# qradiolink/qradiolink

Hardware: AMD Instinct MI355X
Metric: IQ MSamples/sec through RX demod chain (higher is better)
Workload: dtype f32

## Files before the change

### qradiolink_amd/csrc/engine.cpp

```cpp
#include "host_common.hpp"
#include "firdes.hpp"
#include <algorithm>
#include <cmath>
#include <complex>
#include <cstdio>
#include <cstdlib>
#include <cstring>
#include <memory>
#include <new>
#include <string>
#include <mutex>
#include <set>
#include <vector>

using namespace qrl;

static thread_local std::string g_last_error;
int qrl_set_error(int code, const std::string& msg) { g_last_error = msg; return code; }

namespace qrl {
static thread_local bool t_launch_error = false;
hipError_t dyn_lds_limit(const void* kernel, int bytes)
{
    static std::mutex mu;
// ... 120 lines not shown
std::vector<float2> to_f2(const std::vector<std::complex<float>>& v)
{
    std::vector<float2> r(v.size());
    for (size_t i = 0; i < v.size(); ++i) r[i] = make_float2(v[i].real(), v[i].imag());
    return r;
}

struct DecimStage {
    bool used = false, mfma = false, pl = false, pm = false;
    int D = 1, Jpad = 0, variant = DECIM_R4_J12, nt = 0, S = 0;
    DevBuf<float> taps;
    DevBuf<float2> edge, edge_b; uint32_t edge_len = 0;
    int alloc_edge(int B, bool two = false) {
        if (!pl && !pm) return QRL_OK;
        edge_len = (uint32_t)(pm ? decim_pm_edge_len(nt, D) : decim_pl_edge_len(nt, D));
        if (!edge_len) return QRL_OK;
        if (int r = edge.alloc((size_t)B * edge_len)) return r;
        return two ? edge_b.alloc((size_t)B * edge_len) : QRL_OK;
    }
    int plan(const std::vector<float>& h, int D_) {
        used = true; D = D_; nt = (int)h.size();
        if (decim_uses_pm(nt, D)) {
            pm = true;
            return taps.upload(decim_pm_layout(h, D));
        }
        if (decim_uses_pl(nt, D)) {
            pl = true;
            return taps.upload(decim_pl_layout(h, D));
        }
        if (decim_uses_mfma(nt, D)) {
            mfma = true;
// ... 3 lines not shown
            return taps.upload(g);
        }
        const int J = (nt + D - 1) / D;
        const size_t kLds2 = 80 * 1024;
        auto pad = [&](int v) { const int jc = decim_jc(v); return (J + jc - 1) / jc * jc; };
        variant = -1;
        if (J <= 10 && decim_lds_bytes(D, pad(DECIM_R2_J10), DECIM_R2_J10) <= kLds2) variant = DECIM_R2_J10;
        else if (J > 36 && J <= 44 && decim_lds_bytes(D, 44, DECIM_R4_J44) <= kLds2) variant = DECIM_R4_J44;
        else if (decim_lds_bytes(D, pad(DECIM_R4_J12), DECIM_R4_J12) <= kLds2) variant = DECIM_R4_J12;
        else variant = DECIM_R1_J14;
        Jpad = pad(variant);
        if (decim_lds_bytes(D, Jpad, variant) > 160 * 1024) return QRL_ERR_ARG;
        return taps.upload(decim_layout(h, D, Jpad));
    }
    uint32_t lookback() const { return pm ? decim_pm_lookback(nt, D) : pl ? (uint32_t)(((nt + D - 1) / D + 1) * D) : mfma ? (uint32_t)(nt + D) : (uint32_t)(Jpad * D); }
    int launch(DecimParams& p, int B, hipStream_t s, int parity = 0) const {
        p.nt = nt;
        float2* e = parity && edge_b.p ? edge_b.p : edge.p;
        if (pm) { p.pl_taps = taps.p; p.pl_edge = e; p.pl_edge_stride = edge_len; p.pl_edge_cap = edge_len; return launch_decim_pm(p, B, s); }
        if (pl) { p.pl_taps = taps.p; p.pl_edge = e; p.pl_edge_stride = edge_len; p.pl_edge_cap = edge_len; return launch_decim_pl(p, B, s); }
        if (mfma) { p.gtab = taps.p; p.S = S; return launch_decim_mfma(p, B, s); }
        launch_decim(p, B, variant, s);
        return 0;
    }
};

}

struct qrl_demod {
    qrl_ctx* ctx = nullptr;
    qrl_demod_config cfg{};
    hipStream_t stream = nullptr;
    bool own_stream = false;
    hipStream_t tail = nullptr;
    hipStream_t fecs = nullptr;
    hipEvent_t ev_q[2] = {nullptr, nullptr}, ev_fec[2] = {nullptr, nullptr}; bool q_valid[2] = {false, false};
    bool grouped = false, grouped_capable = false, fec_deferred = false; FecParams fec_pending{}; int fec_pending_slot = 0;
    DevBuf<uint64_t> qp_snap;
    hipEvent_t ev_ff = nullptr, ev_tail = nullptr;
    hipStream_t pre = nullptr; hipEvent_t ev_pre = nullptr, ev_fe[2] = {nullptr, nullptr}; bool fe_valid[2] = {false, false}; bool pre_pending = false;
    bool input_resident = false;
    hipEvent_t ev_user[4] = {nullptr, nullptr, nullptr, nullptr};
    bool tail_pending = false;
    bool qpsk_fll = false, fsk4_disc = false;
    bool m17 = false;
    DevBuf<float2> s2g, disc4_taps; DevBuf<float> sym4_taps; int disc4_nt = 0, sym4_nt = 0;
    bool fll_slim = false;
    bool d2f_capable = false, d2f = false; DevBuf<float> d2f_taps;
    bool overlap = false, overlap_capable = false; hipEvent_t ev_tail2[2] = {nullptr, nullptr}; bool tail2_valid[2] = {false, false}; uint64_t call_no = 0;
    enum Family { F_2FSK, F_GMSK, F_QPSK, F_DMR, F_4FSK, F_BPSK, F_DSSS, F_ANALOG } fam = F_2FSK;
    int branches = 2;

    int fe_decim = 1, interp = 1, decim = 1, target = 0, sps_eff = 0;
    bool fm = false;

    DecimStage fe;
// ... 448 lines not shown
{
    if (n > cfg.max_chunk) return qrl_set_error(QRL_ERR_TOO_BIG, "n exceeds max_chunk");
    if ((reinterpret_cast<uintptr_t>(iq) & 15u) || (stride & 1u)) return qrl_set_error(QRL_ERR_ARG, "iq must be 16-byte aligned, stride even");
    const int B = cfg.batch;
    uint32_t* counts = (out && out->counts) ? out->counts : counts_scratch.p;
    hipStream_t cs = overlap ? tail : stream;
    const int slot = (int)(call_no & 1);
    if (overlap) {
        if (tail2_valid[slot]) HIPCHK(hipStreamWaitEvent(stream, ev_tail2[slot], 0));
    } else {
        HIPCHK(hipMemsetAsync(counts, 0, (size_t)B * 4 * sizeof(uint32_t), stream));
    }
    if (loops_family() && q_valid[slot]) HIPCHK(hipStreamWaitEvent(stream, ev_q[slot], 0));
    if (grouped && q_valid[slot ^ 1]) HIPCHK(hipStreamWaitEvent(stream, ev_q[slot ^ 1], 0));
    if (pre_pending) { HIPCHK(hipStreamWaitEvent(stream, ev_pre, 0)); pre_pending = false; }
    const bool use_pre = pre && input_resident;
    const float2* in = reinterpret_cast<const float2*>(iq);
    const float2* hist_old = hist_flip ? hist_b.p : hist_a.p;
    float2* hist_new = hist_flip ? hist_a.p : hist_b.p;

    const uint64_t n_in0 = n_in, n_in1 = n_in + n;
    uint64_t n1_0 = n1, n1_1 = n1;
    RingC r1{s1.p, s1_mask}, r2{s2.p, s2_mask}, r2l{s2l.p, s2_mask}, r2f{s2f.p, s2_mask};
    RingF r2d{s2d.p, s2_mask}, r3{s3.p, s2_mask};

    hipEvent_t ev0 = nullptr, ev1 = nullptr;
    if (profiling) {
        HIPCHK(hipEventCreate(&ev0)); HIPCHK(hipEventCreate(&ev1));
        HIPCHK(hipEventRecord(ev0, stream));
    }
    if (fe.used) {
        n1_1 = decim_count(n_in1, 1, fe_decim);
        DecimParams p{};
        p.in = in; p.in_stride = stride; p.n0 = n_in0; p.n = (uint32_t)n;
        p.hist = hist_old; p.hist_len = hist_len;
        p.out = r1; p.m0 = n1_0; p.m_count = (uint32_t)(n1_1 - n1_0);
        p.taps = fe.taps.p; p.D = fe.D; p.Jpad = fe.Jpad;
        p.rot_enable = 1; rot.fill(p);
        if (use_pre) { p.pre_stream = pre; p.pre_event = ev_pre; }
        if (fe.launch(p, B, stream, use_pre ? slot : 0)) return qrl_set_error(QRL_ERR_HIP, "front-end launch: hipFuncSetAttribute failed");
    }
    if (profiling && fe.used) { HIPCHK(hipEventRecord(ev1, stream)); prof_events.emplace_back(ev0, ev1); }
    const uint64_t src0 = fe.used ? n1_0 : n_in0, src1 = fe.used ? n1_1 : n_in1;
    const uint64_t n2_0 = n2, n2_1 = decim_count(src1, interp, decim);
    if (interp == 1) {
        DecimParams p{};
        if (fe.used) { p.in = nullptr; p.in_ring = r1; }
        else { p.in = in; p.in_stride = stride; p.hist = hist_old; p.hist_len = hist_len;
               p.rot_enable = 1; rot.fill(p); }
        p.n0 = src0; p.n = (uint32_t)(src1 - src0);
        p.out = r2; p.m0 = n2_0; p.m_count = (uint32_t)(n2_1 - n2_0);
        p.taps = first.taps.p; p.D = first.D; p.Jpad = first.Jpad;
        if (d2f) {
            const bool sd = cfg.enable_side_outputs && out;
            Dec2FirParams f{};
            f.d = p; f.taps = d2f_taps.p; f.out = RingC{s2f.p, s2_mask};
            f.port = sd && out->filtered ? reinterpret_cast<float2*>(out->filtered) : nullptr;
            f.port_cap = sd ? out->filtered_cap : 0;
            f.counts = counts;
            launch_dec2_fir(f, B, stream);
        } else {
            if (use_pre && !fe.used) { p.pre_stream = pre; p.pre_event = ev_pre; }
            if (first.launch(p, B, stream, use_pre && !fe.used ? slot : 0)) return qrl_set_error(QRL_ERR_HIP, "first-stage launch: hipFuncSetAttribute failed");
        }
    } else {
        ResampParams p{};
        if (fe.used) { p.in = nullptr; p.in_ring = r1; }
        else { p.in = in; p.in_stride = stride; p.hist = hist_old; p.hist_len = hist_len;
               p.rot_enable = 1; rot.fill(p); }
        p.n0 = src0; p.n = (uint32_t)(src1 - src0);
        p.out = r2; p.q0 = n2_0; p.q_count = (uint32_t)(n2_1 - n2_0);
        p.taps = rs_taps.p; p.I = interp; p.D = decim; p.Jp = rs_Jp;
        if (fam == F_DMR && !m17) {
            const bool sd = cfg.enable_side_outputs && out;
            p.port = sd && out->filtered ? reinterpret_cast<float2*>(out->filtered) : nullptr;
            p.port_cap = sd ? out->filtered_cap : 0;
            p.port_counts = counts;
// ... 7 lines not shown
        if (fe.used) { p.in = nullptr; p.in_ring = r1; }
        else { p.in = in; p.in_stride = stride; p.hist = hist_old; p.hist_len = hist_len;
               p.rot_enable = 1; rot.fill(p); }
        p.n0 = src0; p.n = (uint32_t)(src1 - src0);
        p.out = RingC{s_scope.p, scope_mask}; p.m0 = n_scope; p.m_count = (uint32_t)(ns_1 - n_scope);
        p.taps = scope.taps.p; p.D = scope.D; p.Jpad = scope.Jpad;
        if (scope.launch(p, B, stream)) return qrl_set_error(QRL_ERR_HIP, "scope launch: hipFuncSetAttribute failed");
        launch_ring_store(RingC{s_scope.p, scope_mask}, n_scope, (uint32_t)(ns_1 - n_scope), scope_out, scope_cap, scope_counts, B, stream);
        n_scope = ns_1;
    }
    {
        HistParams h{};
        h.in = in; h.in_stride = stride; h.n0 = n_in0; h.n = (uint32_t)n;
        h.hist_old = hist_old; h.hist_new = hist_new; h.hist_len = hist_len;
        h.rot_enable = 1; rot.fill(h);
        if (pre) { HIPCHK(hipEventRecord(ev_fe[slot], stream)); fe_valid[slot] = true; }
        if (use_pre) {
            if (fe_valid[slot ^ 1]) HIPCHK(hipStreamWaitEvent(pre, ev_fe[slot ^ 1], 0));
            launch_hist_save(h, B, pre);
            HIPCHK(hipEventRecord(ev_pre, pre));
            pre_pending = true;
        } else launch_hist_save(h, B, stream);
        hist_flip = !hist_flip;
    }
    if (overlap) {
        HIPCHK(hipEventRecord(ev_ff, stream));
        HIPCHK(hipStreamWaitEvent(tail, ev_ff, 0));
        HIPCHK(hipMemsetAsync(counts, 0, (size_t)B * 4 * sizeof(uint32_t), tail));
    }
    const uint32_t c2 = (uint32_t)(n2_1 - n2_0);
    const bool side = cfg.enable_side_outputs && out;
    if (fam == F_DSSS || fam == F_ANALOG) {
        if (int rr = fam == F_DSSS ? dsss_stages(n2_0, n2_1, out, counts, side) : analog_stages(n2_0, n2_1, out, counts, side)) return rr;
        HIPCHK(hipGetLastError());
        if (take_launch_error()) return QRL_ERR_HIP;
        n_in = n_in1; n1 = n1_1; n2 = n2_1; ++call_no;
        return QRL_OK;
// ... 373 lines not shown
            if (std::getenv("QRL_CU_MAIN")) { if ((r0 = create_role_stream(&d->stream, 0, "MAIN"))) return r0; }
            else if (std::getenv("QRL_MAIN_PRIO_LOW")) {
                int plo = 0, phi = 0;
                (void)hipDeviceGetStreamPriorityRange(&plo, &phi);
                HIPCHK(hipStreamCreateWithPriority(&d->stream, hipStreamNonBlocking, plo));
            }
            else HIPCHK(hipStreamCreateWithFlags(&d->stream, hipStreamNonBlocking));
            d->own_stream = true;
        }
        int lo = 0, hi = 0;
        (void)hipDeviceGetStreamPriorityRange(&lo, &hi);
        int r1;
        if ((r1 = create_role_stream(&d->tail, hi, "TAIL")) || (r1 = create_role_stream(&d->fecs, lo, "FEC"))) return r1;
        if (d->own_stream && !std::getenv("QRL_NO_PRE")) { if ((r1 = create_role_stream(&d->pre, 0, "PRE"))) return r1; }
    }
    HIPCHK(hipEventCreateWithFlags(&d->ev_ff, hipEventDisableTiming));
    HIPCHK(hipEventCreateWithFlags(&d->ev_pre, hipEventDisableTiming));
    for (auto& e : d->ev_fe) HIPCHK(hipEventCreateWithFlags(&e, hipEventDisableTiming));
    HIPCHK(hipEventCreateWithFlags(&d->ev_tail, hipEventDisableTiming));
    for (auto& e : d->ev_tail2) HIPCHK(hipEventCreateWithFlags(&e, hipEventDisableTiming));
    for (auto& e : d->ev_q) HIPCHK(hipEventCreateWithFlags(&e, hipEventDisableTiming));
    for (auto& e : d->ev_fec) HIPCHK(hipEventCreateWithFlags(&e, hipEventDisableTiming));
    int r = d->build();
    if (r) return r;
    *outp = d.release();
    return QRL_OK;
}
void qrl_demod_destroy(qrl_demod* d) { if (d) { (void)d->sync_all(); delete d; } }

int qrl_demod_reset(qrl_demod* d)
// ... 58 lines not shown
        d->tail2_valid[0] = d->tail2_valid[1] = false;
        return QRL_OK;
    case QRL_OPT_FLL_SLIM:
        if (int rs = d->sync_all()) return rs;
        d->fll_slim = value != 0;
        return QRL_OK;
    case QRL_OPT_GROUPED:
        if (value != 0 && !d->grouped_capable) return qrl_set_error(QRL_ERR_ARG, "the grouped order exists for the gr_demod_qpsk chain only");
        if (int rs = d->sync_all()) return rs;
        d->grouped = value != 0;
        return QRL_OK;
    case QRL_OPT_INPUT_RESIDENT: {
        if (int rs = d->sync_all()) return rs;
        if (value != 0 && d->pre) {
            DecimStage& st = d->fe.used ? d->fe : d->first;
            if (st.edge_len && !st.edge_b.p) if (int r = st.edge_b.alloc((size_t)d->cfg.batch * st.edge_len)) return qrl_set_error(r, "edge scratch");
        }
        d->input_resident = value != 0;
        return QRL_OK;
    }
    case QRL_OPT_UNFUSED_DEC2:
        if (!d->d2f_capable) return qrl_set_error(QRL_ERR_ARG, "this chain has no fused 1:2 decimator + shaping filter");
        if (d->n_in != 0) return qrl_set_error(QRL_ERR_STATE, "QRL_OPT_UNFUSED_DEC2 can only be set before the first sample (the two forms carry different state)");
        d->d2f = value == 0;
        return QRL_OK;
    default:
        return qrl_set_error(QRL_ERR_ARG, "unknown option");
    }
}
int qrl_demod_out_caps(const qrl_demod* d, size_t n, size_t* fcap, size_t* ccap, size_t* bcap)
{
// ... 118 lines not shown
    return QRL_OK;
}
int qrl_demod_set_agc(qrl_demod* d, float attack, float decay)
{
    if (!d || d->fam != qrl_demod::F_ANALOG || (d->an_kind != 1 && d->an_kind != 3)) return QRL_ERR_ARG;
    d->an_attack = attack; d->an_decay = decay;
    return QRL_OK;
}
int qrl_demod_process(qrl_demod* d, const float* iq, size_t stride, size_t n, const qrl_demod_out* out)
{
    if (!d || (!iq && n)) return QRL_ERR_ARG;
    HIPCHK(hipSetDevice(d->ctx->device));
    (void)take_launch_error();
    return d->process(iq, stride, n, out);
}
int qrl_demod_sync(qrl_demod* d)
{
    if (!d) return QRL_ERR_ARG;
    if (int rs = d->sync_all()) return rs;
    return QRL_OK;
}
void* qrl_demod_stream(qrl_demod* d) { return d ? d->stream : nullptr; }
int qrl_demod_internal_streams(qrl_demod* d, void* out[3])
{
    if (!d || !out) return QRL_ERR_ARG;
    out[0] = d->stream; out[1] = d->tail; out[2] = d->fecs;
    return QRL_OK;
}

int qrl_demod_profile(qrl_demod* d, int enable)
// ... 71 lines not shown
```

### qradiolink_amd/csrc/engine.hpp

```cpp
#pragma once
#include <hip/hip_runtime.h>
#include <stdint.h>
#include <vector>

namespace qrl {

hipError_t dyn_lds_limit(const void* kernel, int bytes);
bool take_launch_error();

int create_role_stream(hipStream_t* s, int priority, const char* role);

struct RingC { float2* p; uint32_t mask; };
struct RingF { float* p; uint32_t mask; };
struct RingB { uint8_t* p; uint32_t mask; };

template <class Pp>
__device__ __forceinline__ void rot_select(Pp& c, const Pp& p, uint32_t b)
{
    c = p; c.rot_acc = p.rot_acc_s[b]; c.rot_inc = p.rot_inc_s[b]; c.rot_lo = p.rot_lo + (size_t)b * 512;
}
#define ROT_VIEW(T, PS, P, SRC, B) T P##_ps_; if constexpr (PS) rot_select(P##_ps_, SRC, (uint32_t)(B)); const T& P = (PS) ? P##_ps_ : SRC
std::vector<float2> rot_fine_table(uint64_t inc);
void launch_rot_ps_advance(uint64_t* acc, const uint64_t* inc, int B, uint64_t delta, hipStream_t s);
void launch_rot_ps_fill(uint64_t* acc, uint64_t* inc, float2* lo, int B, int set_acc, uint64_t acc0, uint64_t inc0, const float2* lo0, hipStream_t s);
// ... 7 lines not shown
    uint64_t m0; uint32_t m_count;
    const float* taps;
    int D, Jpad;
    int rot_enable; uint64_t rot_acc; uint64_t rot_inc; uint64_t rot_nbase; const float2* rot_lo;
    uint32_t tiles;
    const float* gtab; int S; int nt; uint32_t magic_blk, magic_seg;
    uint32_t tpw, nchunks; int nhi; int dbg;
    int nld;
    int hist_raw;
    uint32_t out_row_mul_m1, out_row_add;
    const float* pl_taps; int pl_J; uint32_t pl_S, pl_nseg, pl_batch; uint64_t pl_m_begin, pl_m_end;
    int pl_E, pl_R; const float* pl_hraw;
    float2* pl_edge; uint32_t pl_edge_stride, pl_edge_cap; uint64_t pl_edge_ms, pl_edge_me;
    hipStream_t pre_stream; hipEvent_t pre_event;
    const uint64_t* rot_acc_s; const uint64_t* rot_inc_s;
};
struct HistParams {
    const float2* in; size_t in_stride; uint64_t n0; uint32_t n;
    const float2* hist_old; float2* hist_new; uint32_t hist_len;
    int rot_enable; uint64_t rot_acc; uint64_t rot_inc; uint64_t rot_nbase; const float2* rot_lo;
    const uint64_t* rot_acc_s; const uint64_t* rot_inc_s;
};
void launch_decim(const DecimParams& p, int batch, int variant, hipStream_t s);
struct Dec2FirParams { DecimParams d; const float* taps; RingC out; float2* port; size_t port_cap; uint32_t* counts; };
bool dec2_fir_supported(int nt1, int D, int nt2);
uint32_t dec2_fir_lookback();
std::vector<float> dec2_fir_table(const std::vector<float>& h1, const std::vector<float>& h2);
void launch_dec2_fir(const Dec2FirParams& p, int batch, hipStream_t s);
void launch_hist_save(const HistParams& p, int batch, hipStream_t s);
size_t decim_lds_bytes(int D, int Jpad, int variant);
enum { DECIM_R4_J44 = 0, DECIM_R4_J12 = 1, DECIM_R2_J10 = 2, DECIM_R1_J14 = 3 };
int decim_jc(int variant);
bool decim_uses_mfma(int nt, int D);
int decim_mfma_steps(int nt, int D);
int decim_mfma_na(int nt, int D);
int decim_mfma_hpn(int nt, int D);
size_t decim_mfma_lds_bytes(int nt, int D);
int launch_decim_mfma(const DecimParams& p, int batch, hipStream_t s);
void decim_mfma_prof_read(unsigned long long* out8);
void decim_mfma_prof_enable(int on);
bool decim_uses_pl(int nt, int D);
size_t decim_pl_edge_len(int nt, int D);
std::vector<float> decim_pl_layout(const std::vector<float>& h, int D);
int launch_decim_pl(const DecimParams& p, int batch, hipStream_t s);
bool decim_uses_pm(int nt, int D);
size_t decim_pm_edge_len(int nt, int D);
uint32_t decim_pm_lookback(int nt, int D);
std::vector<float> decim_pm_layout(const std::vector<float>& h, int D);
int launch_decim_pm(const DecimParams& p, int batch, hipStream_t s);

struct ResampParams {
    const float2* in; size_t in_stride; uint64_t n0; uint32_t n;
    const float2* hist; uint32_t hist_len;
    RingC in_ring;
    RingC out;
    uint64_t q0; uint32_t q_count;
    const float* taps;
    int I, D, Jp;
    int rot_enable; uint64_t rot_acc; uint64_t rot_inc; uint64_t rot_nbase; const float2* rot_lo;
    float2* port; size_t port_cap; uint32_t* port_counts;
    const uint64_t* rot_acc_s; const uint64_t* rot_inc_s;
};
void launch_resamp(const ResampParams& p, int batch, hipStream_t s);

// ... 249 lines not shown
```

### qradiolink_amd/csrc/kernels_decim_pl.hip

```cpp
#include <vector>
#include <cstdlib>
#include <mutex>
#include "devmath.hpp"
#include "engine.hpp"

namespace qrl {

typedef float v2f __attribute__((ext_vector_type(2)));
typedef float f32x4_pm __attribute__((ext_vector_type(4)));


__device__ __forceinline__ float pl_dpp_ror8(float v)
{
    return __uint_as_float(__builtin_amdgcn_update_dpp(0u, __float_as_uint(v), 0x128 , 0xf, 0xf, true));
}
__device__ __forceinline__ float pl_dpp_xor4(float v)
{
    unsigned r = __builtin_amdgcn_update_dpp(0u, __float_as_uint(v), 0x104 , 0xf, 0x5, false);
    r = __builtin_amdgcn_update_dpp(r, __float_as_uint(v), 0x114 , 0xf, 0xa, false);
    return __uint_as_float(r);
}
template <int CTRL>
__device__ __forceinline__ float pl_dpp_quad(float v)
{
// ... 77 lines not shown
        : [R] "=&v"(R), [C] "=&v"(C), [L] "=&v"(L), [H] "=&v"(H)
        : [z0] "v"(z[0]), [z1] "v"(z[1]), [z2] "v"(z[2]), [z3] "v"(z[3]));
}
__device__ __forceinline__ void pm_glds16(const void* gsrc, uint32_t lds_dst)
{
    unsigned keep;
    asm volatile("s_mov_b32 %0, m0\n\ts_mov_b32 m0, %2\n\ts_nop 0\n\tglobal_load_lds_dwordx4 %1, off nt\n\ts_mov_b32 m0, %0"
                 : "=&s"(keep) : "v"(gsrc), "s"(lds_dst) : "memory");
}
typedef const __attribute__((address_space(3))) v2f* pm_lds_f2;
__device__ __forceinline__ float2 pm_lds(uint32_t addr)
{
    const v2f v = *(pm_lds_f2)(uintptr_t)addr;
    return make_float2(v.x, v.y);
}
__device__ __forceinline__ uint32_t pm_lds_addr(const void* p) { return (uint32_t)(uintptr_t)(const __attribute__((address_space(3))) void*)p; }
template <int N> __device__ __forceinline__ void pm_wait_vm() { asm volatile("s_waitcnt vmcnt(%0)" :: "n"(N) : "memory"); }
__device__ __forceinline__ void pm_wait_vm_dyn(uint32_t allowed)
{
    switch (allowed) {
    case 0: pm_wait_vm<0>(); break;   case 1: pm_wait_vm<1>(); break;   case 2: pm_wait_vm<2>(); break;   case 3: pm_wait_vm<3>(); break;
    case 4: pm_wait_vm<4>(); break;   case 5: pm_wait_vm<5>(); break;   case 6: pm_wait_vm<6>(); break;   case 7: pm_wait_vm<7>(); break;
    case 8: pm_wait_vm<8>(); break;   case 9: pm_wait_vm<9>(); break;   case 10: pm_wait_vm<10>(); break; case 11: pm_wait_vm<11>(); break;
    case 12: pm_wait_vm<12>(); break; case 13: pm_wait_vm<13>(); break; case 14: pm_wait_vm<14>(); break; default: pm_wait_vm<15>(); break;
    }
}

#ifndef QRL_PM_ABL
#define QRL_PM_ABL 0
#endif
#ifdef QRL_PM_PROF
// ... 17 lines not shown
    float2 (*t_hi_all)[NHI] = reinterpret_cast<float2 (*)[NHI]>(t_lo + 512);
    const int tid = threadIdx.x, lane = tid & 63;
    const int wave = __builtin_amdgcn_readfirstlane(tid >> 6);
    if constexpr (!PS) {
        for (int k = tid; k < 512; k += NW * 64) t_lo[k] = P.rot_lo[k];
    } else {
        const uint32_t u0 = blockIdx.x * (uint32_t)NW, nreg0 = P.pl_nseg * P.pl_batch;
        const uint32_t b0 = u0 < nreg0 ? u0 / P.pl_nseg : 0u;
        for (int k = tid; k < 512; k += NW * 64) t_lo[k] = P.rot_lo[(size_t)b0 * 512 + k];
    }

    const uint32_t unit = blockIdx.x * (uint32_t)NW + (uint32_t)wave;
    const uint32_t B = P.pl_batch;
    const uint32_t nreg = P.pl_nseg * B;
    const bool edge = unit >= nreg;
    const uint32_t nsg = P.pl_nseg ? P.pl_nseg : 1u;
    const uint32_t b = edge ? unit - nreg : unit / nsg, seg = edge ? 0u : unit - b * nsg;
    const int D = P.D;
    const uint64_t ms = edge ? P.pl_edge_ms : P.pl_m_begin + (uint64_t)seg * P.pl_S;
    const bool active = edge ? (b < B && P.pl_edge_me > P.pl_edge_ms) : (!PS || ms < P.pl_m_end);
    const uint64_t me = edge ? P.pl_edge_me : (ms + P.pl_S < P.pl_m_end ? ms + P.pl_S : P.pl_m_end);
    const int64_t cfs = (int64_t)ms - (J - 1);
    const int64_t G0 = cfs >= 0 ? cfs / 16 : -((-cfs + 15) / 16);
    const int ngrp = active ? (int)((int64_t)((me - 1) / 16) - G0) + 1 : 0;
    const int64_t i_first_s = (G0 * 16 - 1) * (int64_t)D + 1;
    const uint64_t i_first = (uint64_t)i_first_s;
    uint64_t r_acc = P.rot_acc, r_inc = P.rot_inc;
    if constexpr (PS) {
        const uint32_t bs = b < B ? b : 0u;
        r_acc = P.rot_acc_s[bs]; r_inc = P.rot_inc_s[bs];
    }
    uint32_t kb0 = edge ? 0u : (uint32_t)((i_first - P.rot_nbase) >> 9);
    if (active) t_hi_all[wave][lane] = edge ? make_float2(1.f, 0.f) : sincos_turn(r_acc + ((uint64_t)(kb0 + (uint32_t)lane) << 9) * r_inc);
    __syncthreads();
    if (!active) return;

    float a[NT][NS];
#pragma unroll
    for (int t = 0; t < NT; ++t)
#pragma unroll
        for (int s = 0; s < NS; ++s) a[t][s] = P.pl_taps[(t * NS + s) * 64 + lane];
    const int q = lane >> 4, nn = lane & 15;
    float a1[NT];
#pragma unroll
    for (int t = 0; t < NT; ++t) a1[t] = K1 ? __shfl(a[t][NS - 1], 4 * q + (nn & 3), 64) : 0.f;
    const unsigned char* rowp = reinterpret_cast<const unsigned char*>(edge ? P.pl_edge + (size_t)b * P.pl_edge_stride : P.in + (size_t)b * P.in_stride);
    const uint64_t off0 = edge ? 0ull : (uint64_t)(i_first - P.n0) * 8ull;
    const uint64_t row_bytes = edge ? (uint64_t)P.pl_edge_stride * 8ull : (uint64_t)P.n * 8ull;
    const uint32_t o0 = (uint32_t)(off0 & 127u);
    const uint64_t a_off = off0 - o0;
    const uint32_t GB = 16u * (uint32_t)D * 8u;
    const uint32_t npieces = (o0 + (uint32_t)ngrp * GB + 1023u) >> 10;
    const uint32_t q_safe = (uint32_t)((row_bytes - a_off) >> 10);
    const uint32_t rbase = pm_lds_addr(ring_all) + (uint32_t)wave * (RP * 1024u);
    const uint32_t tlo_base = pm_lds_addr(t_lo);
    const uint32_t thi_base = pm_lds_addr(t_hi_all) + (uint32_t)wave * (NHI * 8u);
    const unsigned char* gp = rowp + a_off + (size_t)lane * 16;
    const unsigned char* last16 = rowp + row_bytes - 16;
    uint32_t issued = 0;
    auto issue_upto = [&](uint32_t want) {
        while (issued < want) {
            const uint32_t dst = rbase + (issued & (RP - 1)) * 1024u;
            if (issued < q_safe) pm_glds16(gp, dst);
            else pm_glds16(gp < last16 ? gp : last16, dst);
            gp += 1024;
            ++issued;
        }
    };
    const uint32_t k0 = edge ? 0u : (uint32_t)(i_first - P.rot_nbase) - (kb0 << 9);
    const uint32_t tl_mask = edge ? 0u : 4095u;
    const uint32_t lane_byte = ((uint32_t)nn * (uint32_t)D + (uint32_t)q) * 8u;
    const bool last_valid = 4 * (NS - 1) + q < D;
    float2* orow = P.out.p + ((size_t)b * (P.out_row_mul_m1 + 1u) + P.out_row_add) * (P.out.mask + 1u);
    float Cpr = 0.f, Cpi = 0.f;
    f32x4_pm nr1 = {0.f, 0.f, 0.f, 0.f}, ni1 = nr1, nr2 = nr1, ni2 = nr1;

#ifdef QRL_PM_PROF
    unsigned long long pc[8] = {0, 0, 0, 0, 0, 0, 0, 0};
    unsigned long long tprev = __builtin_readcyclecounter();
#endif
    issue_upto(npieces < RP ? npieces : RP);
    uint32_t gbytes = o0;
    uint32_t kb8 = (k0 * 8u) + lane_byte;
    uint32_t kg8 = k0 * 8u;
    for (int g = 0; g < ngrp; ++g) {
        if (((kg8 + GB) >> 12) >= (uint32_t)(NHI - 1)) {
            const uint32_t sh = kg8 >> 12;
            kb0 += sh; kg8 -= sh << 12; kb8 -= sh << 12;
            t_hi_all[wave][lane] = edge ? make_float2(1.f, 0.f) : sincos_turn(r_acc + ((uint64_t)(kb0 + (uint32_t)lane) << 9) * r_inc);
        }
        {
            uint32_t need = (gbytes + GB + 1023u) >> 10;
            need = need < npieces ? need : npieces;
            pm_wait_vm_dyn(issued - need);
        }
        PM_STAMP(0);
        float2 x[NS];
        {
            const uint32_t xb = gbytes + lane_byte;
#pragma unroll
            for (int s = 0; s < NS; ++s) x[s] = pm_lds(rbase | ((xb + 32u * (uint32_t)s) & (RP * 1024u - 1u)));
        }
        asm volatile("s_waitcnt lgkmcnt(0)" ::: "memory");
        PM_STAMP(1);
        {
            const uint32_t first_next = (gbytes + GB) >> 10;
            const uint32_t cap = first_next + RP;
            issue_upto(cap < npieces ? cap : npieces);
        }
// ... 64 lines not shown
        const float y = __uint_as_float(w32[0]) + __uint_as_float(w32[1]);
        const int64_t m = (G0 + g) * 16 + nn;
#if QRL_PM_ABL & 1
        if (y == 12345.678f) reinterpret_cast<float*>(orow)[0] = y;
#else
        if (lane < 32 && m >= (int64_t)ms && m < (int64_t)me)
            reinterpret_cast<float*>(orow + ((uint32_t)m & P.out.mask))[q] = y;
#endif
        gbytes += GB;
        kb8 += GB; kg8 += GB;
        PM_STAMP(4);
    }
#ifdef QRL_PM_PROF
    if (lane == 0) { for (int k = 0; k < 5; ++k) atomicAdd(&g_pm_prof[k], pc[k]); atomicAdd(&g_pm_prof[7], (unsigned long long)ngrp); }
#endif
    pm_wait_vm<0>();
}

template <bool PS = false>
__global__ __launch_bounds__(256) void k_decim_pm_gen(const DecimParams P_, uint64_t m_first, uint32_t count)
{
    ROT_VIEW(DecimParams, PS, P, P_, blockIdx.y);
    const uint32_t o = blockIdx.x * 256u + threadIdx.x;
    if (o >= count) return;
    const int b = blockIdx.y;
    const uint64_t m = m_first + o;
    const int D = P.D, nt = P.nt, J = (nt + D - 1) / D;
    const float2* inb = P.in ? P.in + (size_t)b * P.in_stride : nullptr;
    const float2* hb = P.hist ? P.hist + (size_t)b * P.hist_len : nullptr;
    const float2* rb = P.in_ring.p ? P.in_ring.p + (size_t)b * (P.in_ring.mask + 1u) : nullptr;
// ... 491 lines not shown
    }
    const uint32_t S = pm_pick_segment(M, batch, (uint32_t)(wg_per_cu * n_cu * NW), (uint32_t)(J - 1), PS ? (uint32_t)NW : 1u);
    uint32_t nseg = M ? (uint32_t)((M + S - 1) / S) : 0u;
    if (PS) nseg = (nseg + NW - 1) / NW * NW;
    q.pl_S = S;
    q.pl_nseg = nseg;
    const uint32_t units = q.pl_nseg * batch + (edge_unit ? batch : 0u);
    hipLaunchKernelGGL(kern, dim3((units + NW - 1) / NW), dim3(NW * 64), lds, s, q);
    return 0;
}
template <int J, int NS, int RP = QRL_PM_RP, bool K1 = false>
static int pm_launch_main(DecimParams& q, uint64_t M, uint32_t batch, bool edge_unit, hipStream_t s)
{
    return q.rot_acc_s ? pm_launch_main_k<J, NS, RP, K1, true>(q, M, batch, edge_unit, s) : pm_launch_main_k<J, NS, RP, K1, false>(q, M, batch, edge_unit, s);
}
int launch_decim_pm(const DecimParams& p, int batch, hipStream_t s)
{
    if (p.m_count == 0) return 0;
    const int D = p.D, nt = p.nt, NS = (D + 3) / 4;
    const int J = pm_kernel_lags(nt, D);
    DecimParams q = p;
    q.pl_J = J; q.pl_E = 1; q.pl_R = 1;
    q.pl_hraw = p.pl_taps + (size_t)pm_tiles(J) * NS * 64;
    const uint64_t m_end = p.m0 + p.m_count;
    auto gen = [&](uint64_t first, uint64_t last) {
        if (last > first) hipLaunchKernelGGL(p.rot_acc_s ? k_decim_pm_gen<true> : k_decim_pm_gen<false>, dim3((uint32_t)((last - first + 255) / 256), batch), dim3(256), 0, s, q, first, (uint32_t)(last - first));
    };
    const bool dma_ok = p.in && p.rot_enable && (reinterpret_cast<uintptr_t>(p.in) & 15u) == 0 && (p.in_stride & 1u) == 0 && (p.n & 1u) == 0 &&
                        p.pl_edge && (reinterpret_cast<uintptr_t>(p.pl_edge) & 15u) == 0 && (p.pl_edge_stride & 1u) == 0;
    if (!dma_ok) { gen(p.m0, m_end); return 0; }
    const uint64_t qb = p.n0 > 1 ? (p.n0 - 1 + D - 1) / D : 0;
    uint64_t m_main = (qb + 1 + 15) / 16 * 16 + (uint64_t)(J - 1);
    if (m_main < p.m0) m_main = p.m0 + (uint64_t)((((J - 1) % 16) - (int)(p.m0 % 16) + 16) % 16);
    const uint64_t c_max = (p.n0 + p.n - 1) / D;
    uint64_t m_tail = c_max + 1 < m_end ? c_max + 1 : m_end;
    if (m_tail < p.m0) m_tail = p.m0;
    if (m_main > m_tail) m_main = m_tail;
    bool edge_unit = false;
    if (m_main > p.m0) {
        const int64_t cfs = (int64_t)p.m0 - (J - 1);
        const int64_t G0 = cfs >= 0 ? cfs / 16 : -((-cfs + 15) / 16);
        const int64_t i0 = (G0 * 16 - 1) * (int64_t)D + 1;
        const int64_t i_last = (int64_t)(m_main - 1) * D;
        const int64_t len = ((i_last - i0 + 1) + 1) & ~(int64_t)1;
        if (len <= (int64_t)p.pl_edge_cap) {
            hipLaunchKernelGGL(p.rot_acc_s ? k_pl_edge_stage<true> : k_pl_edge_stage<false>, dim3((uint32_t)((len + 255) / 256), batch), dim3(256), 0, p.pre_stream ? p.pre_stream : s, q, i0, (uint32_t)len);
            if (p.pre_stream) { (void)hipEventRecord(p.pre_event, p.pre_stream); (void)hipStreamWaitEvent(s, p.pre_event, 0); }
            q.pl_edge_ms = p.m0; q.pl_edge_me = m_main;
            edge_unit = true;
        } else gen(p.m0, m_main);
    }
    gen(m_tail, m_end);
    if (m_main >= m_tail && !edge_unit) return 0;
    q.pl_m_begin = m_main; q.pl_m_end = m_tail;
    q.pl_batch = (uint32_t)batch;
    const uint64_t M = m_tail - m_main;
    const uint32_t Bn = (uint32_t)batch;
    if (J == 9) return pm_launch_main<9, 13>(q, M, Bn, edge_unit, s);
    if (J > 16) {
#ifndef QRL_PM_NO_K1
        if (D == 25 && J == 42) return pm_launch_main<42, 7, QRL_PM_RP_SMALL, true>(q, M, Bn, edge_unit, s);
        if (D == 25) return pm_launch_main<48, 7, QRL_PM_RP_SMALL, true>(q, M, Bn, edge_unit, s);
#endif
        if (J == 42) switch (NS) {
            case 3: return pm_launch_main<42, 3, QRL_PM_RP_SMALL>(q, M, Bn, edge_unit, s);   case 5: return pm_launch_main<42, 5, QRL_PM_RP_SMALL>(q, M, Bn, edge_unit, s);
            case 7: return pm_launch_main<42, 7, QRL_PM_RP_SMALL>(q, M, Bn, edge_unit, s);   case 13: return pm_launch_main<42, 13, 8>(q, M, Bn, edge_unit, s);
            default: return pm_launch_main<42, 25, 16>(q, M, Bn, edge_unit, s);
        }
// ... 15 lines not shown
```

### qradiolink_amd/csrc/kernels_frontend.hip

```cpp
#include "devmath.hpp"
#include "engine.hpp"

namespace qrl {

typedef float v2f __attribute__((ext_vector_type(2)));

__device__ __forceinline__ float2 rot_apply(float2 x, uint64_t k, const float2* t_hi, uint32_t kb0, const float2* t_lo)
{
    const float2 hi = t_hi[(uint32_t)(k >> 9) - kb0];
    const float2 lo = t_lo[(uint32_t)k & 511u];
    return cmul_fma(x, cmul_fma(hi, lo));
}
__device__ __forceinline__ float2 rot_apply_rel(float2 x, uint32_t krel, const float2* t_hi, const float2* t_lo)
{
    return cmul_fma(x, cmul_fma(t_hi[krel >> 9], t_lo[krel & 511u]));
}

__device__ __forceinline__ float2 decim_fetch(const DecimParams& P, int b, int64_t i, const float2* t_hi, uint32_t kb0,
                                              const float2* t_lo)
{
    if (i < 0) return make_float2(0.f, 0.f);
    const uint64_t ui = (uint64_t)i;
    if (P.in) {
        if (ui >= P.n0 + P.n) return make_float2(0.f, 0.f);
// ... 177 lines not shown
    default:           hipLaunchKernelGGL((k_decim<1, 14, true>), grid, block, lds, s, q); break;
    } else switch (variant) {
    case DECIM_R4_J44: hipLaunchKernelGGL((k_decim<4, 44>), grid, block, lds, s, q); break;
    case DECIM_R4_J12: hipLaunchKernelGGL((k_decim<4, 12>), grid, block, lds, s, q); break;
    case DECIM_R2_J10: hipLaunchKernelGGL((k_decim<2, 10>), grid, block, lds, s, q); break;
    default:           hipLaunchKernelGGL((k_decim<1, 14>), grid, block, lds, s, q); break;
    }
}

template <bool PS>
__global__ __launch_bounds__(256) void k_hist(const HistParams P_)
{
    ROT_VIEW(HistParams, PS, P, P_, blockIdx.y);
    const int b = blockIdx.y;
    const uint32_t k = blockIdx.x * 256u + threadIdx.x;
    if (k >= P.hist_len) return;
    const int64_t i = (int64_t)(P.n0 + P.n) - (int64_t)P.hist_len + (int64_t)k;
    float2 x = make_float2(0.f, 0.f);
    if (i >= (int64_t)P.n0) {
        x = P.in[(size_t)b * P.in_stride + (size_t)((uint64_t)i - P.n0)];
        if (P.rot_enable) {
            const uint64_t kk = (uint64_t)i - P.rot_nbase;
            const float2 hi = sincos_turn(P.rot_acc + ((kk >> 9) << 9) * P.rot_inc);
            x = cmul_fma(x, cmul_fma(hi, P.rot_lo[(uint32_t)kk & 511u]));
        }
    } else if (i >= 0) {
        const uint64_t d = P.n0 - (uint64_t)i;
        if (d <= P.hist_len) x = P.hist_old[(size_t)b * P.hist_len + (P.hist_len - (uint32_t)d)];
    }
    P.hist_new[(size_t)b * P.hist_len + k] = x;
}
void launch_hist_save(const HistParams& p, int batch, hipStream_t s)
{
    if (p.hist_len == 0) return;
    dim3 grid((p.hist_len + 255) / 256, batch), block(256);
    if (p.rot_acc_s) hipLaunchKernelGGL(k_hist<true>, grid, block, 0, s, p);
    else hipLaunchKernelGGL(k_hist<false>, grid, block, 0, s, p);
}

__device__ __forceinline__ float2 resamp_fetch(const ResampParams& P, int b, int64_t i)
{
    if (i < 0) return make_float2(0.f, 0.f);
    const uint64_t ui = (uint64_t)i;
    if (P.in) {
        if (ui >= P.n0 + P.n) return make_float2(0.f, 0.f);
        if (ui >= P.n0) {
            float2 x = P.in[(size_t)b * P.in_stride + (size_t)(ui - P.n0)];
            if (P.rot_enable) {
                const uint64_t kk = ui - P.rot_nbase;
                const float2 hi = sincos_turn(P.rot_acc + ((kk >> 9) << 9) * P.rot_inc);
// ... 268 lines not shown
```

Baseline: 525,700.

## Fuse history save and edge staging into the PM decimator kernel

When the IQ-facing decimation stage uses the PM kernel, the main kernel now writes the rotated history tail itself. The edge unit also reads directly from the previous history buffer and the input instead of from a separately staged scratch buffer. This removes the separate edge-stage and history-save kernel launches, along with the pre-stream event juggling. The cost is extra rare-lane work inside the hot kernel, more complex index arithmetic, and a new env flag (QRL_FE_HELPERS) that restores the old helper-kernel path.

```diff
diff --git a/qradiolink_amd/csrc/engine.cpp b/qradiolink_amd/csrc/engine.cpp
--- a/qradiolink_amd/csrc/engine.cpp
+++ b/qradiolink_amd/csrc/engine.cpp
@@ -158,7 +158,7 @@
     int alloc_edge(int B, bool two = false) {
         if (!pl && !pm) return QRL_OK;
         edge_len = (uint32_t)(pm ? decim_pm_edge_len(nt, D) : decim_pl_edge_len(nt, D));
-        if (!edge_len) return QRL_OK;
+        if (!edge_len || pm) return QRL_OK;
         if (int r = edge.alloc((size_t)B * edge_len)) return r;
         return two ? edge_b.alloc((size_t)B * edge_len) : QRL_OK;
     }
@@ -192,10 +192,18 @@
         return taps.upload(decim_layout(h, D, Jpad));
     }
     uint32_t lookback() const { return pm ? decim_pm_lookback(nt, D) : pl ? (uint32_t)(((nt + D - 1) / D + 1) * D) : mfma ? (uint32_t)(nt + D) : (uint32_t)(Jpad * D); }
-    int launch(DecimParams& p, int B, hipStream_t s, int parity = 0) const {
+    int launch(DecimParams& p, int B, hipStream_t s, int parity = 0) {
         p.nt = nt;
+        if (pm) {
+            p.pl_taps = taps.p; p.pl_edge = nullptr; p.pl_edge_stride = edge_len; p.pl_edge_cap = edge_len;
+            if (edge_len && decim_pm_needs_scratch(p)) {
+                DevBuf<float2>& eb = parity ? edge_b : edge;
+                if (!eb.p && eb.alloc((size_t)B * edge_len)) return -1;
+                p.pl_edge = eb.p;
+            }
+            return launch_decim_pm(p, B, s);
+        }
         float2* e = parity && edge_b.p ? edge_b.p : edge.p;
-        if (pm) { p.pl_taps = taps.p; p.pl_edge = e; p.pl_edge_stride = edge_len; p.pl_edge_cap = edge_len; return launch_decim_pm(p, B, s); }
         if (pl) { p.pl_taps = taps.p; p.pl_edge = e; p.pl_edge_stride = edge_len; p.pl_edge_cap = edge_len; return launch_decim_pl(p, B, s); }
         if (mfma) { p.gtab = taps.p; p.S = S; return launch_decim_mfma(p, B, s); }
         launch_decim(p, B, variant, s);
@@ -218,6 +226,7 @@
     hipEvent_t ev_ff = nullptr, ev_tail = nullptr;
     hipStream_t pre = nullptr; hipEvent_t ev_pre = nullptr, ev_fe[2] = {nullptr, nullptr}; bool fe_valid[2] = {false, false}; bool pre_pending = false;
     bool input_resident = false;
+    bool fe_helpers = false;
     hipEvent_t ev_user[4] = {nullptr, nullptr, nullptr, nullptr};
     bool tail_pending = false;
     bool qpsk_fll = false, fsk4_disc = false;
@@ -696,7 +705,10 @@
     if (loops_family() && q_valid[slot]) HIPCHK(hipStreamWaitEvent(stream, ev_q[slot], 0));
     if (grouped && q_valid[slot ^ 1]) HIPCHK(hipStreamWaitEvent(stream, ev_q[slot ^ 1], 0));
     if (pre_pending) { HIPCHK(hipStreamWaitEvent(stream, ev_pre, 0)); pre_pending = false; }
-    const bool use_pre = pre && input_resident;
+    DecimStage* const iq_stage = fe.used ? &fe : interp == 1 && !d2f ? &first : nullptr;
+    const bool self_hist = iq_stage && iq_stage->pm && !fe_helpers;
+    const bool use_pre = pre && input_resident && !self_hist;
+    uint32_t hist_from = hist_len;
     const float2* in = reinterpret_cast<const float2*>(iq);
     const float2* hist_old = hist_flip ? hist_b.p : hist_a.p;
     float2* hist_new = hist_flip ? hist_a.p : hist_b.p;
@@ -719,6 +731,8 @@
         p.out = r1; p.m0 = n1_0; p.m_count = (uint32_t)(n1_1 - n1_0);
         p.taps = fe.taps.p; p.D = fe.D; p.Jpad = fe.Jpad;
         p.rot_enable = 1; rot.fill(p);
+        p.fe_helpers = fe_helpers;
+        if (self_hist) { p.hist_new = hist_new; p.hist_done_from = &hist_from; }
         if (use_pre) { p.pre_stream = pre; p.pre_event = ev_pre; }
         if (fe.launch(p, B, stream, use_pre ? slot : 0)) return qrl_set_error(QRL_ERR_HIP, "front-end launch: hipFuncSetAttribute failed");
     }
@@ -743,6 +757,8 @@
             launch_dec2_fir(f, B, stream);
         } else {
             if (use_pre && !fe.used) { p.pre_stream = pre; p.pre_event = ev_pre; }
+            p.fe_helpers = fe_helpers;
+            if (self_hist && !fe.used) { p.hist_new = hist_new; p.hist_done_from = &hist_from; }
             if (first.launch(p, B, stream, use_pre && !fe.used ? slot : 0)) return qrl_set_error(QRL_ERR_HIP, "first-stage launch: hipFuncSetAttribute failed");
         }
     } else {
@@ -780,13 +796,17 @@
         h.in = in; h.in_stride = stride; h.n0 = n_in0; h.n = (uint32_t)n;
         h.hist_old = hist_old; h.hist_new = hist_new; h.hist_len = hist_len;
         h.rot_enable = 1; rot.fill(h);
-        if (pre) { HIPCHK(hipEventRecord(ev_fe[slot], stream)); fe_valid[slot] = true; }
-        if (use_pre) {
-            if (fe_valid[slot ^ 1]) HIPCHK(hipStreamWaitEvent(pre, ev_fe[slot ^ 1], 0));
-            launch_hist_save(h, B, pre);
-            HIPCHK(hipEventRecord(ev_pre, pre));
-            pre_pending = true;
-        } else launch_hist_save(h, B, stream);
+        if (self_hist) {
+            if (hist_from > 0) { h.k_end = hist_from; launch_hist_save(h, B, stream); }
+        } else {
+            if (pre) { HIPCHK(hipEventRecord(ev_fe[slot], stream)); fe_valid[slot] = true; }
+            if (use_pre) {
+                if (fe_valid[slot ^ 1]) HIPCHK(hipStreamWaitEvent(pre, ev_fe[slot ^ 1], 0));
+                launch_hist_save(h, B, pre);
+                HIPCHK(hipEventRecord(ev_pre, pre));
+                pre_pending = true;
+            } else launch_hist_save(h, B, stream);
+        }
         hist_flip = !hist_flip;
     }
     if (overlap) {
@@ -1190,6 +1210,7 @@
         if ((r1 = create_role_stream(&d->tail, hi, "TAIL")) || (r1 = create_role_stream(&d->fecs, lo, "FEC"))) return r1;
         if (d->own_stream && !std::getenv("QRL_NO_PRE")) { if ((r1 = create_role_stream(&d->pre, 0, "PRE"))) return r1; }
     }
+    { const char* e = std::getenv("QRL_FE_HELPERS"); d->fe_helpers = e && std::atoi(e) != 0; }
     HIPCHK(hipEventCreateWithFlags(&d->ev_ff, hipEventDisableTiming));
     HIPCHK(hipEventCreateWithFlags(&d->ev_pre, hipEventDisableTiming));
     for (auto& e : d->ev_fe) HIPCHK(hipEventCreateWithFlags(&e, hipEventDisableTiming));
@@ -1278,7 +1299,7 @@
         if (int rs = d->sync_all()) return rs;
         if (value != 0 && d->pre) {
             DecimStage& st = d->fe.used ? d->fe : d->first;
-            if (st.edge_len && !st.edge_b.p) if (int r = st.edge_b.alloc((size_t)d->cfg.batch * st.edge_len)) return qrl_set_error(r, "edge scratch");
+            if (st.edge_len && !st.pm && !st.edge_b.p) if (int r = st.edge_b.alloc((size_t)d->cfg.batch * st.edge_len)) return qrl_set_error(r, "edge scratch");
         }
         d->input_resident = value != 0;
         return QRL_OK;
@@ -1427,6 +1448,17 @@
     (void)take_launch_error();
     return d->process(iq, stride, n, out);
 }
+int qrl_debug_demod_history(qrl_demod* d, float* host, size_t cap_samples, uint32_t* hist_len_out)
+{
+    if (!d || !hist_len_out) return QRL_ERR_ARG;
+    *hist_len_out = d->hist_len;
+    if (!host) return QRL_OK;
+    const size_t need = (size_t)d->cfg.batch * d->hist_len;
+    if (cap_samples < need) return QRL_ERR_ARG;
+    if (int rs = d->sync_all()) return rs;
+    HIPCHK(hipMemcpy(host, d->hist_flip ? d->hist_b.p : d->hist_a.p, need * sizeof(float2), hipMemcpyDeviceToHost));
+    return QRL_OK;
+}
 int qrl_demod_sync(qrl_demod* d)
 {
     if (!d) return QRL_ERR_ARG;
diff --git a/qradiolink_amd/csrc/engine.hpp b/qradiolink_amd/csrc/engine.hpp
--- a/qradiolink_amd/csrc/engine.hpp
+++ b/qradiolink_amd/csrc/engine.hpp
@@ -45,10 +45,13 @@
     float2* pl_edge; uint32_t pl_edge_stride, pl_edge_cap; uint64_t pl_edge_ms, pl_edge_me;
     hipStream_t pre_stream; hipEvent_t pre_event;
     const uint64_t* rot_acc_s; const uint64_t* rot_inc_s;
+    float2* hist_new; uint32_t* hist_done_from; int fe_helpers;
+    uint32_t pl_edge_direct, pl_edge_hs;
 };
 struct HistParams {
     const float2* in; size_t in_stride; uint64_t n0; uint32_t n;
     const float2* hist_old; float2* hist_new; uint32_t hist_len;
+    uint32_t k_end;
     int rot_enable; uint64_t rot_acc; uint64_t rot_inc; uint64_t rot_nbase; const float2* rot_lo;
     const uint64_t* rot_acc_s; const uint64_t* rot_inc_s;
 };
@@ -79,6 +82,7 @@
 uint32_t decim_pm_lookback(int nt, int D);
 std::vector<float> decim_pm_layout(const std::vector<float>& h, int D);
 int launch_decim_pm(const DecimParams& p, int batch, hipStream_t s);
+bool decim_pm_needs_scratch(const DecimParams& p);
 
 struct ResampParams {
     const float2* in; size_t in_stride; uint64_t n0; uint32_t n;
diff --git a/qradiolink_amd/csrc/kernels_decim_pl.hip b/qradiolink_amd/csrc/kernels_decim_pl.hip
--- a/qradiolink_amd/csrc/kernels_decim_pl.hip
+++ b/qradiolink_amd/csrc/kernels_decim_pl.hip
@@ -115,7 +115,17 @@
     const v2f v = *(pm_lds_f2)(uintptr_t)addr;
     return make_float2(v.x, v.y);
 }
+__device__ __forceinline__ void pm_lds_put(uint32_t addr, float2 v)
+{
+    *(__attribute__((address_space(3))) v2f*)(uintptr_t)addr = v2f{v.x, v.y};
+}
 __device__ __forceinline__ uint32_t pm_lds_addr(const void* p) { return (uint32_t)(uintptr_t)(const __attribute__((address_space(3))) void*)p; }
+__device__ __forceinline__ uint32_t pm_rare_lane()
+{
+    uint32_t z = 0u;
+    asm volatile("" : "+s"(z));
+    return __builtin_amdgcn_mbcnt_hi(~0u, __builtin_amdgcn_mbcnt_lo(~0u, z));
+}
 template <int N> __device__ __forceinline__ void pm_wait_vm() { asm volatile("s_waitcnt vmcnt(%0)" :: "n"(N) : "memory"); }
 __device__ __forceinline__ void pm_wait_vm_dyn(uint32_t allowed)
 {
@@ -163,6 +173,7 @@
     const uint32_t B = P.pl_batch;
     const uint32_t nreg = P.pl_nseg * B;
     const bool edge = unit >= nreg;
+    const bool edir = edge && P.pl_edge_direct;
     const uint32_t nsg = P.pl_nseg ? P.pl_nseg : 1u;
     const uint32_t b = edge ? unit - nreg : unit / nsg, seg = edge ? 0u : unit - b * nsg;
     const int D = P.D;
@@ -180,7 +191,9 @@
         r_acc = P.rot_acc_s[bs]; r_inc = P.rot_inc_s[bs];
     }
     uint32_t kb0 = edge ? 0u : (uint32_t)((i_first - P.rot_nbase) >> 9);
-    if (active) t_hi_all[wave][lane] = edge ? make_float2(1.f, 0.f) : sincos_turn(r_acc + ((uint64_t)(kb0 + (uint32_t)lane) << 9) * r_inc);
+    const uint64_t kbn = (P.n0 - P.rot_nbase) >> 9;
+    if (active) t_hi_all[wave][lane] = edge ? (edir && lane >= 32 ? sincos_turn(r_acc + ((kbn + (uint64_t)(lane - 32)) << 9) * r_inc) : make_float2(1.f, 0.f))
+                                            : sincos_turn(r_acc + ((uint64_t)(kb0 + (uint32_t)lane) << 9) * r_inc);
     __syncthreads();
     if (!active) return;
 
@@ -193,11 +206,11 @@
     float a1[NT];
 #pragma unroll
     for (int t = 0; t < NT; ++t) a1[t] = K1 ? __shfl(a[t][NS - 1], 4 * q + (nn & 3), 64) : 0.f;
-    const unsigned char* rowp = reinterpret_cast<const unsigned char*>(edge ? P.pl_edge + (size_t)b * P.pl_edge_stride : P.in + (size_t)b * P.in_stride);
+    const unsigned char* rowp = reinterpret_cast<const unsigned char*>(edge && !edir ? P.pl_edge + (size_t)b * P.pl_edge_stride : P.in + (size_t)b * P.in_stride);
     const uint64_t off0 = edge ? 0ull : (uint64_t)(i_first - P.n0) * 8ull;
-    const uint64_t row_bytes = edge ? (uint64_t)P.pl_edge_stride * 8ull : (uint64_t)P.n * 8ull;
-    const uint32_t o0 = (uint32_t)(off0 & 127u);
-    const uint64_t a_off = off0 - o0;
+    const uint64_t row_bytes = edge && !edir ? (uint64_t)P.pl_edge_stride * 8ull : (uint64_t)P.n * 8ull;
+    const uint32_t o0 = edir ? (uint32_t)((int64_t)P.pl_edge_hs - ((int64_t)P.n0 - i_first_s)) * 8u : (uint32_t)(off0 & 127u);
+    const uint64_t a_off = off0 - (edir ? 0u : o0);
     const uint32_t GB = 16u * (uint32_t)D * 8u;
     const uint32_t npieces = (o0 + (uint32_t)ngrp * GB + 1023u) >> 10;
     const uint32_t q_safe = (uint32_t)((row_bytes - a_off) >> 10);
@@ -206,11 +219,17 @@
     const uint32_t thi_base = pm_lds_addr(t_hi_all) + (uint32_t)wave * (NHI * 8u);
     const unsigned char* gp = rowp + a_off + (size_t)lane * 16;
     const unsigned char* last16 = rowp + row_bytes - 16;
+    const unsigned char* hist_end = reinterpret_cast<const unsigned char*>(P.hist + (size_t)(b + 1u) * P.hist_len);
     uint32_t issued = 0;
     auto issue_upto = [&](uint32_t want) {
         while (issued < want) {
             const uint32_t dst = rbase + (issued & (RP - 1)) * 1024u;
-            if (issued < q_safe) pm_glds16(gp, dst);
+            if (edir) {
+                const int32_t d = (int32_t)(issued * 128u + 2u * pm_rare_lane()) - (int32_t)P.pl_edge_hs;
+                const unsigned char* src = d < 0 ? hist_end + (int64_t)d * 8 : rowp + (size_t)d * 8u;
+                pm_glds16(d >= 0 && src > last16 ? last16 : src, dst);
+            }
+            else if (issued < q_safe) pm_glds16(gp, dst);
             else pm_glds16(gp < last16 ? gp : last16, dst);
             gp += 1024;
             ++issued;
@@ -221,6 +240,15 @@
     const uint32_t lane_byte = ((uint32_t)nn * (uint32_t)D + (uint32_t)q) * 8u;
     const bool last_valid = 4 * (NS - 1) + q < D;
     float2* orow = P.out.p + ((size_t)b * (P.out_row_mul_m1 + 1u) + P.out_row_add) * (P.out.mask + 1u);
+    const int64_t hw0 = (int64_t)(P.n0 + P.n) - (int64_t)P.hist_len;
+    int g_hist = 0x7fffffff;
+    if (!edge && P.hist_new) {
+        const int64_t c_lo = hw0 <= 0 ? 0 : (hw0 + D - 1) / D;
+        const int64_t c_w = c_lo > (int64_t)ms ? c_lo : (int64_t)ms;
+        if ((int64_t)me > c_lo) g_hist = c_w / 16 > G0 ? (int)(c_w / 16 - G0) : 0;
+    }
+    const float2* rot_lo_b = P.rot_lo + (PS ? (size_t)(b < B ? b : 0u) * 512 : (size_t)0);
+    float2* hist_row = P.hist_new + (size_t)b * P.hist_len;
     float Cpr = 0.f, Cpi = 0.f;
     f32x4_pm nr1 = {0.f, 0.f, 0.f, 0.f}, ni1 = nr1, nr2 = nr1, ni2 = nr1;
 
@@ -242,6 +270,33 @@
             uint32_t need = (gbytes + GB + 1023u) >> 10;
             need = need < npieces ? need : npieces;
             pm_wait_vm_dyn(issued - need);
+        }
+        if (edir) {
+            const int64_t ig0 = i_first_s + (int64_t)g * 16 * D;
+            for (uint32_t j = pm_rare_lane(); j < 16u * (uint32_t)D; j += 64u) {
+                const int64_t r = ig0 + (int64_t)j - (int64_t)P.n0;
+                if (r >= 0 && r < (int64_t)P.n) {
+                    const uint32_t la = rbase | ((gbytes + 8u * j) & (RP * 1024u - 1u));
+                    const uint64_t kk = P.n0 + (uint64_t)r - P.rot_nbase;
+                    const float2 hi = t_hi_all[wave][32u + (uint32_t)((kk >> 9) - kbn)];
+                    pm_lds_put(la, cmul_fma(pm_lds(la), cmul_fma(hi, rot_lo_b[(uint32_t)kk & 511u])));
+                }
+            }
+        }
+        if (g >= g_hist) {
+            const uint32_t lr = pm_rare_lane(), nr = lr & 15u, qr = lr >> 4, lbyte = (nr * (uint32_t)D + qr) * 8u;
+            const int64_t c = (G0 + g) * 16 + (int64_t)nr;
+            const bool own = c >= (int64_t)ms && c < (int64_t)me;
+            const int32_t kq = (int32_t)((c - 1) * D + 1 + (int64_t)qr - hw0);
+#pragma unroll 1
+            for (int s = 0; s < NS; ++s) {
+                const int32_t k = kq + 4 * s;
+                if (own && 4 * s + (int)qr < D && k >= 0) {
+                    const uint32_t kk = kb8 + 32u * (uint32_t)s;
+                    const float2 raw = pm_lds(rbase | ((gbytes + lbyte + 32u * (uint32_t)s) & (RP * 1024u - 1u)));
+                    hist_row[k] = cmul_fma(raw, cmul_fma(pm_lds(thi_base + ((kk >> 12) << 3)), pm_lds(tlo_base + (kk & 4095u))));
+                }
+            }
         }
         PM_STAMP(0);
         float2 x[NS];
@@ -336,6 +391,15 @@
 #ifdef QRL_PM_PROF
     if (lane == 0) { for (int k = 0; k < 5; ++k) atomicAdd(&g_pm_prof[k], pc[k]); atomicAdd(&g_pm_prof[7], (unsigned long long)ngrp); }
 #endif
+    if (!edge && P.hist_new && me == P.pl_m_end) {
+        const int64_t e_blk = (int64_t)(me - 1) * D + 1;
+        const float2* in_row = P.in + (size_t)b * P.in_stride;
+        for (int64_t i = (e_blk > hw0 ? e_blk : hw0) + (int64_t)pm_rare_lane(); i < (int64_t)(P.n0 + P.n); i += 64) {
+            const uint64_t kk = (uint64_t)i - P.rot_nbase;
+            const float2 hi = sincos_turn(r_acc + ((kk >> 9) << 9) * r_inc);
+            hist_row[i - hw0] = cmul_fma(in_row[(uint64_t)i - P.n0], cmul_fma(hi, rot_lo_b[(uint32_t)kk & 511u]));
+        }
+    }
     pm_wait_vm<0>();
 }
 
@@ -857,37 +921,74 @@
 {
     return q.rot_acc_s ? pm_launch_main_k<J, NS, RP, K1, true>(q, M, batch, edge_unit, s) : pm_launch_main_k<J, NS, RP, K1, false>(q, M, batch, edge_unit, s);
 }
-int launch_decim_pm(const DecimParams& p, int batch, hipStream_t s)
-{
-    if (p.m_count == 0) return 0;
-    const int D = p.D, nt = p.nt, NS = (D + 3) / 4;
-    const int J = pm_kernel_lags(nt, D);
-    DecimParams q = p;
-    q.pl_J = J; q.pl_E = 1; q.pl_R = 1;
-    q.pl_hraw = p.pl_taps + (size_t)pm_tiles(J) * NS * 64;
-    const uint64_t m_end = p.m0 + p.m_count;
-    auto gen = [&](uint64_t first, uint64_t last) {
-        if (last > first) hipLaunchKernelGGL(p.rot_acc_s ? k_decim_pm_gen<true> : k_decim_pm_gen<false>, dim3((uint32_t)((last - first + 255) / 256), batch), dim3(256), 0, s, q, first, (uint32_t)(last - first));
-    };
-    const bool dma_ok = p.in && p.rot_enable && (reinterpret_cast<uintptr_t>(p.in) & 15u) == 0 && (p.in_stride & 1u) == 0 && (p.n & 1u) == 0 &&
-                        p.pl_edge && (reinterpret_cast<uintptr_t>(p.pl_edge) & 15u) == 0 && (p.pl_edge_stride & 1u) == 0;
-    if (!dma_ok) { gen(p.m0, m_end); return 0; }
+struct PmPlan {
+    bool dma_ok; int J; uint64_t m_end, m_main, m_tail;
+    bool edge;
+    bool direct;
+    int64_t i0, len; uint32_t hs;
+};
+static PmPlan pm_plan(const DecimParams& p)
+{
+    PmPlan pl{};
+    const int D = p.D;
+    const int J = pl.J = pm_kernel_lags(p.nt, D);
+    pl.m_end = p.m0 + p.m_count;
+    pl.dma_ok = p.in && p.rot_enable && (reinterpret_cast<uintptr_t>(p.in) & 15u) == 0 && (p.in_stride & 1u) == 0 && (p.n & 1u) == 0 && p.n > 0;
+    if (!pl.dma_ok) return pl;
     const uint64_t qb = p.n0 > 1 ? (p.n0 - 1 + D - 1) / D : 0;
     uint64_t m_main = (qb + 1 + 15) / 16 * 16 + (uint64_t)(J - 1);
     if (m_main < p.m0) m_main = p.m0 + (uint64_t)((((J - 1) % 16) - (int)(p.m0 % 16) + 16) % 16);
     const uint64_t c_max = (p.n0 + p.n - 1) / D;
-    uint64_t m_tail = c_max + 1 < m_end ? c_max + 1 : m_end;
+    uint64_t m_tail = c_max + 1 < pl.m_end ? c_max + 1 : pl.m_end;
     if (m_tail < p.m0) m_tail = p.m0;
     if (m_main > m_tail) m_main = m_tail;
-    bool edge_unit = false;
+    pl.m_main = m_main; pl.m_tail = m_tail;
     if (m_main > p.m0) {
         const int64_t cfs = (int64_t)p.m0 - (J - 1);
         const int64_t G0 = cfs >= 0 ? cfs / 16 : -((-cfs + 15) / 16);
-        const int64_t i0 = (G0 * 16 - 1) * (int64_t)D + 1;
+        pl.i0 = (G0 * 16 - 1) * (int64_t)D + 1;
         const int64_t i_last = (int64_t)(m_main - 1) * D;
-        const int64_t len = ((i_last - i0 + 1) + 1) & ~(int64_t)1;
-        if (len <= (int64_t)p.pl_edge_cap) {
-            hipLaunchKernelGGL(p.rot_acc_s ? k_pl_edge_stage<true> : k_pl_edge_stage<false>, dim3((uint32_t)((len + 255) / 256), batch), dim3(256), 0, p.pre_stream ? p.pre_stream : s, q, i0, (uint32_t)len);
+        pl.len = ((i_last - pl.i0 + 1) + 1) & ~(int64_t)1;
+        pl.edge = pl.len <= (int64_t)p.pl_edge_cap;
+        const int64_t hspan = (int64_t)p.n0 - pl.i0, hs = hspan + (hspan & 1);
+        const int64_t span = ((int64_t)((m_main - 1) / 16) - G0 + 1) * 16 * D + 2;
+        pl.direct = pl.edge && !p.fe_helpers && p.hist && (reinterpret_cast<uintptr_t>(p.hist) & 15u) == 0 && (p.hist_len & 1u) == 0 &&
+                    hspan >= 0 && hs <= (int64_t)p.hist_len && span / 512 + 2 <= 32;
+        pl.hs = (uint32_t)hs;
+    }
+    return pl;
+}
+bool decim_pm_needs_scratch(const DecimParams& p)
+{
+    const PmPlan pl = pm_plan(p);
+    return pl.dma_ok && pl.edge && !pl.direct;
+}
+int launch_decim_pm(const DecimParams& p, int batch, hipStream_t s)
+{
+    if (p.hist_done_from) *p.hist_done_from = p.hist_len;
+    if (p.m_count == 0) return 0;
+    const int D = p.D, NS = (D + 3) / 4;
+    const PmPlan pl = pm_plan(p);
+    const int J = pl.J;
+    DecimParams q = p;
+    q.pl_J = J; q.pl_E = 1; q.pl_R = 1;
+    q.pl_hraw = p.pl_taps + (size_t)pm_tiles(J) * NS * 64;
+    q.hist_new = nullptr; q.pl_edge_direct = 0;
+    const uint64_t m_end = pl.m_end;
+    auto gen = [&](uint64_t first, uint64_t last) {
+        if (last > first) hipLaunchKernelGGL(p.rot_acc_s ? k_decim_pm_gen<true> : k_decim_pm_gen<false>, dim3((uint32_t)((last - first + 255) / 256), batch), dim3(256), 0, s, q, first, (uint32_t)(last - first));
+    };
+    if (!pl.dma_ok) { gen(p.m0, m_end); return 0; }
+    const uint64_t m_main = pl.m_main, m_tail = pl.m_tail;
+    bool edge_unit = false;
+    if (m_main > p.m0) {
+        const bool scratch_ok = p.pl_edge && (reinterpret_cast<uintptr_t>(p.pl_edge) & 15u) == 0 && (p.pl_edge_stride & 1u) == 0;
+        if (pl.direct) {
+            q.pl_edge_direct = 1; q.pl_edge_hs = pl.hs;
+            q.pl_edge_ms = p.m0; q.pl_edge_me = m_main;
+            edge_unit = true;
+        } else if (pl.edge && scratch_ok) {
+            hipLaunchKernelGGL(p.rot_acc_s ? k_pl_edge_stage<true> : k_pl_edge_stage<false>, dim3((uint32_t)((pl.len + 255) / 256), batch), dim3(256), 0, p.pre_stream ? p.pre_stream : s, q, pl.i0, (uint32_t)pl.len);
             if (p.pre_stream) { (void)hipEventRecord(p.pre_event, p.pre_stream); (void)hipStreamWaitEvent(s, p.pre_event, 0); }
             q.pl_edge_ms = p.m0; q.pl_edge_me = m_main;
             edge_unit = true;
@@ -895,6 +996,10 @@
     }
     gen(m_tail, m_end);
     if (m_main >= m_tail && !edge_unit) return 0;
+    if (m_tail > m_main && p.hist_new && p.hist_done_from && !p.fe_helpers) {
+        const int64_t hw0 = (int64_t)(p.n0 + p.n) - (int64_t)p.hist_len, sa = (int64_t)(m_main - 1) * D + 1;
+        if (sa - hw0 < (int64_t)p.hist_len) { q.hist_new = p.hist_new; *p.hist_done_from = sa <= hw0 ? 0u : (uint32_t)(sa - hw0); }
+    }
     q.pl_m_begin = m_main; q.pl_m_end = m_tail;
     q.pl_batch = (uint32_t)batch;
     const uint64_t M = m_tail - m_main;
diff --git a/qradiolink_amd/csrc/kernels_frontend.hip b/qradiolink_amd/csrc/kernels_frontend.hip
--- a/qradiolink_amd/csrc/kernels_frontend.hip
+++ b/qradiolink_amd/csrc/kernels_frontend.hip
@@ -215,7 +215,7 @@
     ROT_VIEW(HistParams, PS, P, P_, blockIdx.y);
     const int b = blockIdx.y;
     const uint32_t k = blockIdx.x * 256u + threadIdx.x;
-    if (k >= P.hist_len) return;
+    if (k >= (P.k_end ? P.k_end : P.hist_len)) return;
     const int64_t i = (int64_t)(P.n0 + P.n) - (int64_t)P.hist_len + (int64_t)k;
     float2 x = make_float2(0.f, 0.f);
     if (i >= (int64_t)P.n0) {
@@ -234,7 +234,7 @@
 void launch_hist_save(const HistParams& p, int batch, hipStream_t s)
 {
     if (p.hist_len == 0) return;
-    dim3 grid((p.hist_len + 255) / 256, batch), block(256);
+    dim3 grid(((p.k_end ? p.k_end : p.hist_len) + 255) / 256, batch), block(256);
     if (p.rot_acc_s) hipLaunchKernelGGL(k_hist<true>, grid, block, 0, s, p);
     else hipLaunchKernelGGL(k_hist<false>, grid, block, 0, s, p);
 }
```

Result: no change. 531,200, median of 2 (+1.0%).
